# PolyU-IOR/HPR-LP-C

Measured on AMD Instinct MI355X. Metric: HPR iterations/sec (FP64), higher is better.
Workload: dtype f64

## Files before the change

hpr-lp-c_amd/csrc/abi.cpp:

```cpp
#include <algorithm>
#include <cmath>
#include <cstdlib>
#include <cstring>
#include <memory>
#include <mutex>
#include <iomanip>
#include <iostream>

#include "hprlp_amd.h"
#include "env.h"
#include "dist.h"
#include "presolve.h"
#include "reorder.h"
#include "solver.h"
#include "many.h"
#include "version.h"

using namespace hprlp;

struct hprlp_solver {
    Solver s;
    Comm *comm = nullptr;
    Comm *xcomm = nullptr;
    bool sharded = false;
// ... 1345 lines not shown
    return M.passes;
    GUARD_END(-1)
}

extern "C" int hprlp_tiled_host_check(int m, int n, const int *rowptr, const int *col, int R, int T, double min_dense, long out[6]) {
    try {
        if (m <= 0 || n <= 0 || !rowptr || !col || !out) throw std::runtime_error("bad arguments");
        tiled_host_check(m, n, rowptr, col, R, T, min_dense, out);
        return 0;
    } catch (const std::exception &e) {
        set_last_error(e.what());
        return -1;
    }
}

extern "C" int hprlp_env_switches(char *buf, int cap) {
    int count = 0;
    const EnvEntry *t = env_table(&count);
    std::string d;
    for (int i = 0; i < count; ++i) d += std::string(t[i].name) + "\t" + (t[i].kind == EnvKind::Integrator ? "integrator" : "hook") + "\t" + t[i].what + "\n";
    if (buf && cap > 0) std::snprintf(buf, static_cast<size_t>(cap), "%s", d.c_str());
    return static_cast<int>(d.size());
}

extern "C" int hprlp_solver_time_iterations(hprlp_solver *h, int warmup, int steps, int mode, double *total_ms,
                                            double *xhalf_ms, double *yhalf_ms) {
    GUARD_BEGIN
    Solver &s = h->s;
    if (steps <= 0) throw std::runtime_error("steps must be positive");
    s.run_normal(warmup);
// ... 61 lines not shown
```

hpr-lp-c_amd/csrc/env.cpp:

```cpp
#include "env.h"

#include <cstdlib>
#include <cstring>
#include <stdexcept>

namespace hprlp {

static const EnvEntry kTable[] = {
    {"HPRLP_TEST_HOOKS", EnvKind::Integrator, "1: honour the test hooks below (tests/conftest.py and the tools/ scripts set it)"},
    {"HPRLP_TIMING", EnvKind::Integrator, "wall time of the set-up and solve phases on stderr"},
    {"HPRLP_NO_GRAPH", EnvKind::Integrator, "launch normal iterations eagerly instead of replaying hipGraphs (fall-back)"},
    {"HPRLP_NO_TILED", EnvKind::Integrator, "never build the column-tiled matrix copies: stream kernel everywhere (fall-back)"},
    {"HPRLP_NO_REORDER", EnvKind::Integrator, "no set-up time locality ordering of a large matrix"},
    {"HPRLP_NO_ALLOC_CACHE", EnvKind::Integrator, "do not keep freed device blocks for the next solver of the process"},
    {"HPRLP_DIST_TRANSPORT", EnvKind::Integrator, "shm: hprlp_dist_unique_id names a shared-memory segment (host-staged group of processes on one node) instead of RCCL ids"},
    {"HPRLP_NO_WARM_MODEL", EnvKind::Integrator, "the model constructors do NOT start the HIP runtime / device context / code objects (for a process that forks workers after building its models: a HIP context does not survive fork); the first solve pays for them as in the reference"},
    {"HPRLP_DIST_EXCHANGE", EnvKind::Hook, "sparse | allgather: force the multi-GPU exchange form (same value on every rank)"},
    {"HPRLP_NO_OVERLAP", EnvKind::Integrator, "multi-GPU: shards unsplit, exchange in line on the solver stream"},
    {"HPRLP_DIST_TIMEOUT_S", EnvKind::Integrator, "seconds a rank of the shared-memory transport waits for its peers before it fails (default 120)"},
    {"HPRLP_BATCH_CHUNK", EnvKind::Hook, "solve_batched with 64 or more problems: chunk width of the panels (default 64; narrower chunks map one chunk to each XCD -- measured slower, profiles/r03_tiled_decomposition.md section 6b)"},
    {"HPRLP_BATCH_GRID", EnvKind::Hook, "solve_batched: cap on the row blocks of the normal half-step kernels (read at every call; a small cap makes every workgroup's row loop wrap)"},
    {"HPRLP_BATCH_LAMBDA", EnvKind::Hook, "solve_batched: the batch's lambda_max from the caller (strtod; hand it over as a C99 hex float to keep every bit) instead of 1.01 x the power iteration's estimate (read at every call)"},
    {"HPRLP_COPY_PAUSE_US", EnvKind::Hook, "piece size and pause of the threaded copies of set-up (64 MB, 100 us)"},
    {"HPRLP_COPY_PIECE_MB", EnvKind::Hook, "piece size and pause of the threaded copies of set-up (64 MB, 100 us)"},
// ... 28 lines not shown
    {"HPRLP_PRESOLVE_MAX_LINKS", EnvKind::Hook, "run one presolve stage alone / cut the chain after n links (tests, debugging)"},
    {"HPRLP_PRESOLVE_OFF", EnvKind::Hook, "switch presolve reductions / stages off (any subset; diagnostics)"},
    {"HPRLP_PRESOLVE_ONLY", EnvKind::Hook, "run one presolve stage alone / cut the chain after n links (tests, debugging)"},
    {"HPRLP_REORDER_CLUSTER", EnvKind::Hook, "knobs of the HOST reference path of the ordering (hprlp_locality_ordering): nodes per cluster, refinement sweeps, trimming percentage"},
    {"HPRLP_REORDER_HOST", EnvKind::Hook, "run the clustering of the locality ordering on the host (the reference form; default: on the device)"},
    {"HPRLP_REORDER_SWEEPS", EnvKind::Hook, "knobs of the HOST reference path of the ordering (hprlp_locality_ordering): nodes per cluster, refinement sweeps, trimming percentage"},
    {"HPRLP_REORDER_TRIM", EnvKind::Hook, "knobs of the HOST reference path of the ordering (hprlp_locality_ordering): nodes per cluster, refinement sweeps, trimming percentage"},
    {"HPRLP_SLACK_PIVOT", EnvKind::Hook, "pivot threshold of the costed slack-column substitution (default 0.5 of the row's largest entry)"},
    {"HPRLP_STORE_X", EnvKind::Hook, "every normal x-half reads and stores x (default for matrices with a tiled copy: inside a run of normal iterations x is rebuilt from x_hat and last_x by the next launch instead of travelling through memory)"},
    {"HPRLP_STREAM_NNZ", EnvKind::Hook, "row-block shape of the stream kernel (≤ 64 rows, ≤ 512 nonzeros per wave)"},
    {"HPRLP_STREAM_ROWS", EnvKind::Hook, "row-block shape of the stream kernel (≤ 64 rows, ≤ 512 nonzeros per wave)"},
    {"HPRLP_TILED_ANYWAY", EnvKind::Hook, "attempt the tiled form although neighbouring rows gather from the same lines (<= 0.25 lines per entry) / keep the piece form although an XCD's rows gather from under 3 MB"},
    {"HPRLP_TILED_MIN_COLS", EnvKind::Hook, "fewest columns for the tiled form (default 800 k, 2^19 for lowered super-blocks; 0 when HPRLP_TILED_MIN_ROWS is given)"},
    {"HPRLP_TILED_MIN_DENSE", EnvKind::Hook, "thresholds of the tiled copy (default 32·8192 rows, 0.5 of the entries in staged tiles)"},
    {"HPRLP_TILED_MIN_ROWS", EnvKind::Hook, "thresholds of the tiled copy (default 32·8192 rows, 0.5 of the entries in staged tiles)"},
    {"HPRLP_TILE_COLS", EnvKind::Hook, "force the tile width / super-block height of the tiled copies (default: Solver::choose_sb_rows)"},
    {"HPRLP_TILE_PIECES", EnvKind::Hook, "piece count of the tiled kernel's piece form (default: the chip's workgroup slots when the matrix has at most that many super-blocks; 0 = off)"},
    {"HPRLP_TILE_ROT", EnvKind::Hook, "alignment period of the rotated tile sweeps (default: mean window width of the matrix; 0 = ascending sweeps, i.e. CSR summation order)"},
    {"HPRLP_TILE_ROWS", EnvKind::Hook, "force the tile width / super-block height of the tiled copies (default: Solver::choose_sb_rows)"},
    {"HPRLP_TILE_STAMPS", EnvKind::Hook, "diagnostic instantiation of the piece kernel: shader-clock time per phase of a step on stderr when the solver is destroyed"},
    {"HPRLP_TILE_THREADS", EnvKind::Hook, "build the tiled copies with the host builder (background threads, default min(16, cores)) instead of on the device"},
    {"HPRLP_TILING_CHECK", EnvKind::Hook, "build them with both builders and fail on the first differing array element"},
    {"HPRLP_WG_TIMES", EnvKind::Hook, "diagnostic: per-workgroup wall-clock stamps of the fused tiled kernel on stderr"},
    {"HPRLP_WG_TIMES_DUMP", EnvKind::Hook, "per-workgroup stamps of the normal half-step kernels only, with the CU each ran on; raw table for tools/wgtimes_analyze.py"},
};

const EnvEntry *env_table(int *count) {
    if (count) *count = static_cast<int>(sizeof(kTable) / sizeof(kTable[0]));
    return kTable;
}
// ... 31 lines not shown
```

hpr-lp-c_amd/csrc/kernels.hip:

```cpp
#include "kernels.h"

#include <algorithm>
#include <vector>
#include <cmath>
#include <type_traits>

namespace hprlp {

__device__ __forceinline__ double wave_sum(double v) {
#pragma unroll
    for (int off = 32; off > 0; off >>= 1) v += __shfl_xor(v, off, kWave);
    return v;
}

__device__ __forceinline__ double wave_max(double v) {
#pragma unroll
    for (int off = 32; off > 0; off >>= 1) v = fmax(v, __shfl_xor(v, off, kWave));
    return v;
}

template <int NACC, int NW, int NMAX = 0>
__device__ __forceinline__ void block_store_partials_in(double (&acc)[NACC], double *partials, int stride, double (*red)[NACC > 0 ? NACC : 1]) {
    const int wave = threadIdx.x >> 6, lane = threadIdx.x & 63;
#pragma unroll
// ... 221 lines not shown
#ifndef HPRLP_EPI_NT
#define HPRLP_EPI_NT 2
#endif

template <int ED, int TD, bool REP, bool STAMP = false, bool LOGTERM = false, int TC = kTileCols>
__device__ __forceinline__ void tiled_sweep(const TiledDev &t, int s0, int nst, int first, int count, const double *__restrict__ vec,
                                            int ncols, double *acc, double *ytile, int tid, unsigned long long *stamp = nullptr) {
    constexpr int NT = kTileThreads, R = kTileRows, K = kTileChunk;
    constexpr int TPT = TC / NT;
    static_assert(TC == kTileCols || TC == kTileColsNarrow, "tile width");
    typedef double d2_t __attribute__((ext_vector_type(2)));
    const int lane = tid & 63;
    auto sidx = [&](int i) { i = min(i, count - 1) + first; return s0 + (i < nst ? i : i - nst); };
    int seg = 0, lim = 0;
    int tc0 = 0, tc1 = 0, tc2 = 0, tc3 = 0, tb0 = 0, tb1 = 0, tb2 = 0, tb3 = 0, te0 = 0, te1 = 0, te2 = 0, te3 = 0;
    auto getstep = [&](int k, int &col0, int &eb, int &ee) {
        const int r = min(k, lim - 1) - seg;
        col0 = step_field(tc0, tc1, tc2, tc3, r);
        eb = step_field(tb0, tb1, tb2, tb3, r);
        ee = step_field(te0, te1, te2, te3, r);
    };
    struct Ent {
        d2_t va, vb;
        uint32_t i0, i1, i2;
    };
    typedef uint32_t u3_t __attribute__((ext_vector_type(3), aligned(4)));
    auto issue_entries = [&](Ent &E, int k) {
        int col0, eb, ee_;
        getstep(k, col0, eb, ee_);
        const int e = eb + K * tid;
        const int ee = (e < ee_) ? e : eb;
        E.va = __builtin_nontemporal_load(reinterpret_cast<const d2_t *>(t.tval + ee));
        E.vb = __builtin_nontemporal_load(reinterpret_cast<const d2_t *>(t.tval + ee) + 1);
        const u3_t w = __builtin_nontemporal_load(reinterpret_cast<const u3_t *>(t.tidx3 + (ee / K) * 3));
        E.i0 = w.x;
        E.i1 = w.y;
        E.i2 = w.z;
    };
    typedef double d2u_t __attribute__((ext_vector_type(2), aligned(8)));
    auto issue_tile = [&](double (&tl)[TPT], int k) {
        int col0, eb, ee_;
        getstep(k, col0, eb, ee_);
        static_assert(TPT % 2 == 0, "tile loads come in pairs");
#pragma unroll
        for (int j = 0; j < TPT / 2; ++j) {
            const int p = col0 + 2 * (tid + j * NT);
            const int q = min(p, ncols - 2);
            d2u_t v = *reinterpret_cast<const d2u_t *>(vec + q);
            if (q != p) v.x = v.y;
            tl[2 * j] = v.x;
            tl[2 * j + 1] = v.y;
        }
    };
    auto store_tile = [&](const double (&tl)[TPT]) {
#pragma unroll
        for (int j = 0; j < TPT / 2; ++j) {
            d2_t v;
            v.x = tl[2 * j];
            v.y = tl[2 * j + 1];
            reinterpret_cast<d2_t *>(ytile)[tid + j * NT] = v;
        }
    };
    auto process = [&](const Ent &E, int k) {
        int col0, eb, ee_;
        getstep(k, col0, eb, ee_);
        if (K * tid < ee_ - eb) {
            const double v[K] = {E.va.x, E.va.y, E.vb.x, E.vb.y};
            const uint32_t c0 = E.i0, c1 = E.i1, c2 = E.i2;
            const uint32_t id[K] = {c0 & 0xffffffu, (c0 >> 24) | ((c1 & 0xffffu) << 8), (c1 >> 16) | ((c2 & 0xffu) << 16), c2 >> 8};
            uint32_t rw[K];
            double y[K];
#pragma unroll
            for (int k2 = 0; k2 < K; ++k2) {
                rw[k2] = id[k2] & (R - 1);
                y[k2] = ytile[id[k2] >> kTileRowBits];
            }
            double a[K];
#pragma unroll
            for (int k2 = 0; k2 < K; ++k2) a[k2] = acc[rw[k2]];
            double sk[K], pr[K];
#pragma unroll
            for (int k2 = 0; k2 < K; ++k2) pr[k2] = LOGTERM ? (v[k2] != v[k2] ? 0.0 : v[k2] - y[k2]) : v[k2] * y[k2];
            sk[0] = a[0] + pr[0];
#pragma unroll
// ... 2147 lines not shown
```

hpr-lp-c_amd/csrc/tiled.cpp:

```cpp
#include "tiled.h"
#include "env.h"

#include <algorithm>
#include <cstdlib>
#include <cstring>
#include <string>
#include <thread>
#include <type_traits>

namespace hprlp {

namespace {

struct Local {
    std::vector<int> sb_steps, sb_mid;
    std::vector<TileStep> steps;
    std::vector<char> step_is_rem;
    std::vector<uint32_t> tidx;
    std::vector<int> tperm, rcol, rperm;
    std::vector<uint16_t> rrow;
    long dense = 0, pad = 0;
};

void build_range(int rows, int cols, const int *rp, const int *ci, int sb0, int sb1, Local *L, int R, int T, int rem_cap) {
// ... 266 lines not shown
                if (row_of(k) != sb * R + rrow[e]) throw std::runtime_error("tiled check: a remainder entry in the wrong super-block / row");
            }
        }
    }
    for (long k = 0; k < nnz; ++k)
        if (!seen[k]) throw std::runtime_error("tiled check: an entry is missing");
    if (most_run > kTileLayers * ((static_cast<long>(R) * kTileChunk + kTileStepCap - 1) / kTileStepCap + 1)) throw std::runtime_error("tiled check: too many steps for one tile");
    out[0] = static_cast<long>(h.n_tile);
    out[1] = static_cast<long>(h.n_rem);
    out[2] = static_cast<long>(h.steps.size());
    out[3] = pads;
    out[4] = most_run;
    out[5] = static_cast<long>(1e6 * static_cast<double>(h.dense_entries) / static_cast<double>(nnz));
}

void DeviceTiled::upload(const TiledHost &h, int R, int T, int rem_cap) {
    n_tile = static_cast<long>(h.n_tile);
    n_rem = static_cast<long>(h.n_rem);
    n_steps = static_cast<int>(h.steps.size());
    const int nsb = static_cast<int>(h.sb_mid.size());
    sb_ptr.alloc(h.sb_ptr.size()); sb_ptr.upload(h.sb_ptr.data(), h.sb_ptr.size());
    sb_mid.alloc(h.sb_mid.size()); sb_mid.upload(h.sb_mid.data(), h.sb_mid.size());
    steps.alloc(h.steps.size()); steps.upload(h.steps.data(), h.steps.size());
    tidx.alloc_zero(h.n_tile + 8);
    tperm.alloc(h.n_tile + 8);
    tval.alloc_zero(h.n_tile + 8);
    rcol.alloc_zero(h.n_rem + 8);
    rperm.alloc(h.n_rem + 8);
    rrow.alloc_zero(h.n_rem + 8);
    size_t to = 0, ro = 0;
// ... 8 lines not shown
            HIP_CHECK(hipMemcpy(rrow.p + ro, pc.rrow.data(), pc.rrow.size() * sizeof(uint16_t), hipMemcpyHostToDevice));
        }
        to += pc.tidx.size();
        ro += pc.rcol.size();
    }
    view.valid = true;
    view.R = R;
    view.T = T;
    view.rem_cap = rem_cap;
    view.nsb = nsb;
    view.sb_ptr = sb_ptr.p;
    view.sb_mid = sb_mid.p;
    view.steps = steps.p;
    view.tval = tval.p;
    pack_indices(nullptr);
    view.tidx3 = tidx3.p;
    finish_schedule(nullptr);
}

void DeviceTiled::compare_with(const TiledHost &h) const {
    auto fail = [](const std::string &what) { throw std::runtime_error("tiling check: " + what); };
    if (n_tile != static_cast<long>(h.n_tile)) fail("tile entries " + std::to_string(n_tile) + " vs " + std::to_string(h.n_tile));
    if (n_rem != static_cast<long>(h.n_rem)) fail("remainder entries " + std::to_string(n_rem) + " vs " + std::to_string(h.n_rem));
    if (dense_entries != h.dense_entries || padding != h.padding) fail("dense / padding totals");
    auto same = [&](const char *name, const auto &dbuf, const auto &host) {
        using T = typename std::decay<decltype(host[0])>::type;
        std::vector<T> dev(host.size());
        if (!host.empty()) HIP_CHECK(hipMemcpy(dev.data(), dbuf.p, host.size() * sizeof(T), hipMemcpyDeviceToHost));
        for (size_t i = 0; i < host.size(); ++i)
            if (std::memcmp(&dev[i], &host[i], sizeof(T)) != 0) fail(std::string(name) + " differs at " + std::to_string(i));
    };
    same("sb_ptr", sb_ptr, h.sb_ptr);
    same("sb_mid", sb_mid, h.sb_mid);
    if (static_cast<size_t>(n_steps) != h.steps.size()) fail("step count");
    {
        std::vector<TileStep> dev(h.steps.size());
        if (!dev.empty()) HIP_CHECK(hipMemcpy(dev.data(), steps.p, dev.size() * sizeof(TileStep), hipMemcpyDeviceToHost));
        for (size_t i = 0; i < dev.size(); ++i)
            if (dev[i].col0 != h.steps[i].col0 || dev[i].e_begin != h.steps[i].e_begin || dev[i].e_end != h.steps[i].e_end)
                fail("steps differ at " + std::to_string(i));
    }
    std::vector<uint32_t> a_tidx;
    std::vector<int> a_tperm, a_rcol, a_rperm;
    std::vector<uint16_t> a_rrow;
    for (const TiledHost::Piece &pc : h.pieces) {
        a_tidx.insert(a_tidx.end(), pc.tidx.begin(), pc.tidx.end());
        a_tperm.insert(a_tperm.end(), pc.tperm.begin(), pc.tperm.end());
        a_rcol.insert(a_rcol.end(), pc.rcol.begin(), pc.rcol.end());
        a_rperm.insert(a_rperm.end(), pc.rperm.begin(), pc.rperm.end());
        a_rrow.insert(a_rrow.end(), pc.rrow.begin(), pc.rrow.end());
    }
    {
        std::vector<uint32_t> packed(a_tidx.size() / 4 * 3);
        for (size_t c = 0; c < a_tidx.size() / 4; ++c) {
            const uint32_t e0 = a_tidx[4 * c], e1 = a_tidx[4 * c + 1], e2 = a_tidx[4 * c + 2], e3 = a_tidx[4 * c + 3];
            packed[3 * c] = e0 | (e1 << 24);
            packed[3 * c + 1] = (e1 >> 8) | (e2 << 16);
            packed[3 * c + 2] = (e2 >> 16) | (e3 << 8);
        }
        same("tidx3", tidx3, packed);
    }
    same("tperm", tperm, a_tperm);
    same("rcol", rcol, a_rcol);
    same("rperm", rperm, a_rperm);
    same("rrow", rrow, a_rrow);
}

}
```

hpr-lp-c_amd/csrc/tiled.h:

```cpp
#pragma once

#include <hip/hip_runtime.h>

#include <cstdint>
#include <vector>

#include "common.h"

namespace hprlp {

constexpr int kTileThreads = 512;
constexpr int kTileRows = 8192;
constexpr int kTileCols = 2048;
constexpr int kTileColsNarrow = 1024;
constexpr int kTileChunk = 4;
constexpr int kTileStepCap = kTileThreads * kTileChunk;
constexpr int kTileRemK = 4;
constexpr int kTileRemCap = (kTileThreads - 4) * kTileRemK;
constexpr int kTileRemRun = 16;
#ifndef HPRLP_PB_REM_K
#define HPRLP_PB_REM_K 8
#endif
constexpr int kPbRemK = HPRLP_PB_REM_K;
constexpr int kPbRemCap = kTileThreads * kPbRemK;
constexpr int kPbRowsMax = 4096;
constexpr int kPbRunTabCap = 3072;
constexpr int kTileMaxRow = 1024;
constexpr int kTileDenseMin = 256;
static_assert(kTileRemCap % kTileRemK == 0 && kTileRemCap + (kTileThreads / 64) * 3 / 2 <= kTileCols, "tile buffer too small for the remainder scratch");
constexpr int kTileRowBits = 13;
constexpr int kTileRowsMin = 1024;
static_assert((1 << kTileRowBits) == kTileRows && kTileCols <= (1 << (24 - kTileRowBits)) && kTileChunk == 4,
              "entry codes are 24 bits: 13 of local row, 11 of local column, four per chunk");
inline uint32_t tile_code(int lcol, int row) { return (static_cast<uint32_t>(lcol) << kTileRowBits) | static_cast<uint32_t>(row); }

struct PackLayout {
    int n1 = 0, n2 = 0, n3 = 0, n4 = 0;
    int u3 = 0, u2 = 0, r1 = 0, c2 = 0;
    __host__ __device__ void set(int a1, int a2, int a3, int a4) {
        n1 = a1; n2 = a2; n3 = a3; n4 = a4;
        u3 = n1 < n3 ? n1 : n3;
        c2 = (n2 + 1) / 2;
        const int left = n1 - u3;
        u2 = (n2 & 1) ? (left < 2 ? left : 2) : 0;
        r1 = left - u2;
    }
    __host__ __device__ int entries() const { return kTileChunk * (n4 + n3 + c2 + (r1 + 3) / 4); }
    __host__ __device__ int pos(int L, int j) const {
        if (L == 4) return 4 * j;
// ... 58 lines not shown
    double *parts = nullptr;
    const int4 *side_blk = nullptr;
    int side_nblk = 0;
    const int4 *side_long = nullptr;
    int side_nlong = 0;
    double *side_partial = nullptr;
    const int *side_rows = nullptr;
    double *base = nullptr;
    unsigned long long *stamps = nullptr;
    unsigned long long *wgtimes = nullptr;
    int wg_filter = 0;
    const int *sb_ptr = nullptr;
    const int *sb_mid = nullptr;
    const TileStep *steps = nullptr;
    const double *tval = nullptr;
    const uint32_t *tidx3 = nullptr;
    double *P = nullptr;
    const uint32_t *rq = nullptr;
    int n_groups = 0;
    const int *f_gptr = nullptr;
    const double *f_val = nullptr;
    const int *f_pos = nullptr;
    const uint16_t *f_lcol = nullptr;
    const int *f_rptr = nullptr;
    const int *f_rk = nullptr;
    const int *f_rp = nullptr;
    int f_maxruns = 0;
    const int4 *f_work = nullptr;
    int n_work = 0;
};

// ... 5 lines not shown
        std::vector<int> tperm;
        std::vector<int> rcol, rperm;
        std::vector<uint16_t> rrow;
    };
    std::vector<Piece> pieces;
    size_t n_tile = 0, n_rem = 0;
    long dense_entries = 0;
    long padding = 0;
};

bool build_tiled(int rows, int cols, const int *rowptr, const int *col, TiledHost *out, int min_rows,
                 double min_dense_fraction, int R = kTileRows, int T = kTileCols, int rem_cap = kTileRemCap);

void tiled_host_check(int rows, int cols, const int *rp, const int *ci, int R, int T, double min_dense, long out[6]);

void compact_without_rows(long nnz, int rows, const int *rp_dev, const int *rp_c_dev, const int *col_dev, int *col_c, int *map_c, hipStream_t s);

struct DeviceTiled {
    DBuf<int> sb_ptr, sb_mid, tperm, rperm, rcol;
    DBuf<TileStep> steps;
    DBuf<uint32_t> tidx;
    DBuf<uint32_t> tidx3;
    DBuf<uint16_t> rrow;
    DBuf<double> tval;
    DBuf<double> P, f_val;
    DBuf<uint32_t> rq;
    DBuf<int> f_gptr, f_pos, f_perm;
    DBuf<int> f_rptr, f_rk, f_rp;
    DBuf<int4> f_work;
    DBuf<uint16_t> f_lcol;
    TiledDev view;
    long n_tile = 0, n_rem = 0;
    double rem_top_share = 0.0;
    long dense_entries = 0, padding = 0;
    int n_steps = 0;
    void upload(const TiledHost &h, int R = kTileRows, int T = kTileCols, int rem_cap = kTileRemCap);
    void pack_indices(hipStream_t s);
// ... 25 lines not shown
```

hpr-lp-c_amd/csrc/tiled_build.hip:

```cpp
#include <algorithm>
#include <functional>
#include <cstdlib>
#include <hipcub/hipcub.hpp>

#include <vector>

#include "common.h"
#include "env.h"
#include "kernels.h"
#include "tiled.h"

namespace hprlp {

namespace {

constexpr int K = kTileChunk;
constexpr int kRowBits = kTileRowBits;

__device__ __forceinline__ int row_of_entry(const int *__restrict__ rowptr, int rows, int k) {
    int lo = 0, hi = rows;
    while (hi - lo > 1) {
        const int mid = lo + ((hi - lo) >> 1);
        if (rowptr[mid] <= k) lo = mid;
        else hi = mid;
// ... 271 lines not shown
    rperm[e] = k;
    rcol[e] = col[k];
    rrow[e] = static_cast<uint16_t>(row_of_entry(rowptr, rows, k) % R);
}

__global__ void __launch_bounds__(kThreads) k_rem_steps(int nsb, int rem_cap, const int *__restrict__ sb_mid, const int *__restrict__ rem_before,
                                                       TileStep *__restrict__ steps) {
    const int sb = blockIdx.x * kThreads + threadIdx.x;
    if (sb >= nsb) return;
    const int b = rem_before[sb], e = rem_before[sb + 1];
    for (int p = b, j = 0; p < e; p += rem_cap, ++j) steps[sb_mid[sb] + j] = TileStep{0, p, min(e, p + rem_cap), 0};
}

inline unsigned grid_for(long n) { return static_cast<unsigned>((n + kThreads - 1) / kThreads); }

__global__ void __launch_bounds__(kThreads) k_pack_codes(long nchunk, const uint32_t *__restrict__ code, uint32_t *__restrict__ packed) {
    const long c = static_cast<long>(blockIdx.x) * kThreads + threadIdx.x;
    if (c >= nchunk) return;
    const uint32_t e0 = code[4 * c], e1 = code[4 * c + 1], e2 = code[4 * c + 2], e3 = code[4 * c + 3];
    packed[3 * c] = e0 | (e1 << 24);
    packed[3 * c + 1] = (e1 >> 8) | (e2 << 16);
    packed[3 * c + 2] = (e2 >> 16) | (e3 << 8);
}

}

void DeviceTiled::pack_indices(hipStream_t s) {
    const long nchunk = n_tile / K;
    tidx3.alloc_zero(static_cast<size_t>(nchunk) * 3 + 8);
    if (nchunk > 0) hipLaunchKernelGGL(k_pack_codes, dim3(grid_for(nchunk)), dim3(kThreads), 0, s, nchunk, tidx.p, tidx3.p);
    HIP_CHECK(hipStreamSynchronize(s));
    tidx.release();
}

namespace {

__global__ void __launch_bounds__(kThreads) k_window_widths(int nsb, int T, const int *__restrict__ sb_ptr, const int *__restrict__ sb_mid,
                                                           const TileStep *__restrict__ steps, unsigned long long *__restrict__ out) {
    const int sb = blockIdx.x * kThreads + threadIdx.x;
    if (sb >= nsb) return;
    const int s0 = sb_ptr[sb], smid = sb_mid[sb];
    if (s0 >= smid) return;
    const int w = (steps[smid - 1].col0 - steps[s0].col0) / T + 1;
    atomicAdd(out, static_cast<unsigned long long>(w));
    atomicAdd(out + 1, 1ull);
    int rep = 0;
    for (int s = s0 + 1; s < smid; ++s) rep += steps[s].col0 == steps[s - 1].col0;
    if (rep) atomicAdd(out + 2, static_cast<unsigned long long>(rep));
}

__global__ void __launch_bounds__(kThreads) k_rotation(int nsb, int period, int T, const int *__restrict__ sb_ptr, const int *__restrict__ sb_mid,
                                                      TileStep *__restrict__ steps) {
    const int sb = blockIdx.x * kThreads + threadIdx.x;
    if (sb >= nsb) return;
    const int s0 = sb_ptr[sb], smid = sb_mid[sb];
    if (s0 >= smid) return;
    const int nst = smid - s0;
    const int w0 = steps[s0].col0 / T;
    const long target = static_cast<long>((w0 + period - 1) / period) * period * T;
    int lo = 0, hi = nst;
    while (lo < hi) {
        const int mid = (lo + hi) >> 1;
// ... 236 lines not shown

    dense_entries = static_cast<long>(tot[0]);
    padding = static_cast<long>(tot[1]);
    n_steps = total_steps;
    view = TiledDev();
    view.valid = true;
    view.R = R;
    view.T = T;
    view.rem_cap = rem_cap;
    view.nsb = nsb;
    view.sb_ptr = sb_ptr.p;
    view.sb_mid = sb_mid.p;
    view.steps = steps.p;
    view.tval = tval.p;
    pack_indices(s);
    view.tidx3 = tidx3.p;
    finish_schedule(s);
    return true;
}


namespace {

__global__ void __launch_bounds__(kThreads) k_far_step_of(int nsb, const int *__restrict__ sb_ptr, const int *__restrict__ sb_mid,
                                                         TileStep *__restrict__ steps, const uint16_t *__restrict__ rrow,
                                                         int *__restrict__ step_of, int *__restrict__ sb_of, bool mark) {
    const int sb = blockIdx.x;
    if (sb >= nsb) return;
    for (int s = sb_mid[sb]; s < sb_ptr[sb + 1]; ++s) {
        const TileStep st = steps[s];
        if (threadIdx.x == 0) steps[s].col0 = 0;
// ... 414 lines not shown
```

hpr-lp-c_amd/hprlp.py:

```python
import ctypes as C
import os
import time
import weakref

import numpy as np

_HERE = os.path.dirname(os.path.abspath(__file__))
_ROOT = os.path.dirname(_HERE)
LIB_PATH = os.environ.get("HPRLP_LIB") or os.path.join(_ROOT, "lib", "libhprlp.so")

c_int_p = C.POINTER(C.c_int)
c_dbl_p = C.POINTER(C.c_double)


class CParameters(C.Structure):
    _fields_ = [
        ("max_iter", C.c_int), ("stop_tol", C.c_double), ("time_limit", C.c_double),
        ("device_number", C.c_int), ("check_iter", C.c_int),
        ("CUSPARSE_spmv", C.c_bool), ("autotune_verbose", C.c_bool), ("use_CR_scaling", C.c_bool),
        ("use_Ruiz_scaling", C.c_bool), ("use_Pock_Chambolle_scaling", C.c_bool),
        ("use_bc_scaling", C.c_bool), ("use_presolve", C.c_bool),
    ]


# ... 742 lines not shown
        out = (C.c_long * 8)()
        self._chk(lib().hprlp_solver_info(self.h, out))
        keys = ("m", "n", "nnz", "blocks_A", "blocks_AT", "grid_y", "grid_x", "tiled")
        d = dict(zip(keys, [int(v) for v in out]))
        d["reordered"] = bool(d["tiled"] & 8)
        d["tiled"] &= 7
        return d

    def describe(self):
        buf = C.create_string_buffer(2048)
        L = lib()
        L.hprlp_solver_describe.argtypes = [C.c_void_p, C.c_char_p, C.c_int]
        self._chk(L.hprlp_solver_describe(self.h, buf, 2048))
        return buf.value.decode()

    def form_facts(self):
        L = lib()
        L.hprlp_solver_form_facts.argtypes = [C.c_void_p, C.c_int, C.POINTER(CFormFacts)]
        out = {}
        for which, name in enumerate(("A", "A^T")):
            buf = (CFormFacts * 2)()
            n = L.hprlp_solver_form_facts(self.h, which, buf)
            self._chk(min(n, 0))
            out[name] = [_struct_dict(buf[i]) for i in range(n)]
        return out

    def run(self, max_trace=4096):
        res = CResults()
        trace = (CTraceRow * max_trace)()
        nt = C.c_int(0)
# ... 91 lines not shown
```

include/hprlp_amd.h:

```cpp
#ifndef HPRLP_AMD_H
#define HPRLP_AMD_H

#include "HPRLP.h"

#ifdef __cplusplus
extern "C" {
#endif

typedef struct hprlp_solver hprlp_solver;

typedef struct hprlp_trace_row {
    int iter, restart_flag;
    double err_Rp, err_Rd, primal_obj, dual_obj, gap, kkt, sigma, current_gap, lambda_max;
} hprlp_trace_row;

const char *hprlp_last_error(void);
const char *hprlp_backend(void);
int hprlp_warmup(int device);
int hprlp_warmup_seconds(double out[4]);

void hprlp_release_device_cache(void);
int hprlp_alloc_cache_selftest(void);

hprlp_solver *hprlp_solver_create(const LP_info_cpu *model, const HPRLP_parameters *param);
// ... 117 lines not shown
                                                   hprlp_local_group *group);

typedef struct hprlp_presolve hprlp_presolve;
hprlp_presolve *hprlp_presolve_run(const LP_info_cpu *model);
const LP_info_cpu *hprlp_presolve_reduced(const hprlp_presolve *p);
int hprlp_presolve_stats(const hprlp_presolve *p, int out[16]);
int hprlp_presolve_postsolve(const hprlp_presolve *p, const double *xr, const double *yr, const double *zr, double *x,
                             double *y, double *z);
int hprlp_presolve_forward(const hprlp_presolve *p, const double *x, const double *y, double *xr, double *yr);
void hprlp_presolve_free(hprlp_presolve *p);
int hprlp_original_kkt(const LP_info_cpu *model, const double *x, const double *y, const double *z, double out[5]);

int hprlp_locality_ordering(int m, int n, const int *rowptr, const int *col, int *row_new2old, int *col_new2old, double out[6]);
int hprlp_row_block_plan(int m, int n, const int *rowptr, const int *col, int with_cuts, long out[6]);
int hprlp_tiled_host_check(int m, int n, const int *rowptr, const int *col, int R, int T, double min_dense, long out[6]);

typedef struct hprlp_form_built {
    long ok;
    long n_pieces, dense_entries, n_rem;
    double rem_top_share;
} hprlp_form_built;
typedef struct hprlp_form_facts {
    long rows, cols, nnz, longest_row;
    double long_row_share;
    double line_density;
    double xcd_gather_bytes;
    long sb_rows, slots;
    double min_dense_override;
    long sharded;
    long heaviest_block;
// ... 14 lines not shown
} hprlp_form_hooks;
typedef struct hprlp_form_decision {
    int min_rows, min_cols;
    double min_dense;
    int route;
    int side_tried;
    int kept;
    int form;
    int why;
    int long_rows_alone;
    int all_remainder_wanted;
    char note[96];
} hprlp_form_decision;
int hprlp_form_select(const hprlp_form_facts *facts, const hprlp_form_hooks *hooks, hprlp_form_decision *out);
int hprlp_solver_form_facts(hprlp_solver *s, int which, hprlp_form_facts out[2]);

#ifdef __cplusplus
}
#endif
#endif
```

Measured before the change: 787.0.

## Compress tiled-matrix entry codes to 10 bytes per chunk where shapes fit

Replaces the 12-byte packed index triple per chunk of four entries with a split layout: an 8-byte lo/hi word plus a 2-byte word, and a 2-byte extra word read only for steps marked wide. A compact encoding stores four 11-bit local columns plus the row pattern (ascending small deltas, repeated rows, pairs) when it fits. Each step gets a wide flag in the low bit of col0. The goal is to cut index bytes streamed by the tiled SpMV, at the cost of extra decode ALU, more load instructions, and a per-step choice of mode.

```diff
diff --git a/hpr-lp-c_amd/csrc/abi.cpp b/hpr-lp-c_amd/csrc/abi.cpp
--- a/hpr-lp-c_amd/csrc/abi.cpp
+++ b/hpr-lp-c_amd/csrc/abi.cpp
@@ -1383,6 +1383,30 @@
     }
 }
 
+extern "C" int hprlp_tile_codes_host_check(int m, int n, const int *rowptr, const int *col, int R, int T, double min_dense, int force_wide, long out[5]) {
+    try {
+        if (m <= 0 || n <= 0 || !rowptr || !col || !out) throw std::runtime_error("bad arguments");
+        tile_codes_host_check(m, n, rowptr, col, R, T, min_dense, force_wide != 0, out);
+        return 0;
+    } catch (const std::exception &e) {
+        set_last_error(e.what());
+        return -1;
+    }
+}
+
+extern "C" int hprlp_solver_tile_codes(hprlp_solver *h, long out[8]) {
+    GUARD_BEGIN
+    if (!h || !out) throw std::runtime_error("null solver / output");
+    Solver &s = h->s;
+    s.finish_tiling();
+    for (int w = 0; w < 2; ++w) {
+        const DeviceMatrix &M = w ? s.AT : s.A;
+        for (int i = 0; i < 4; ++i) out[4 * w + i] = M.view.tiled.valid ? M.tiled.code_stats[i] : 0;
+    }
+    return 0;
+    GUARD_END(-1)
+}
+
 extern "C" int hprlp_env_switches(char *buf, int cap) {
     int count = 0;
     const EnvEntry *t = env_table(&count);
diff --git a/hpr-lp-c_amd/csrc/env.cpp b/hpr-lp-c_amd/csrc/env.cpp
--- a/hpr-lp-c_amd/csrc/env.cpp
+++ b/hpr-lp-c_amd/csrc/env.cpp
@@ -66,6 +66,7 @@
     {"HPRLP_TILED_MIN_COLS", EnvKind::Hook, "fewest columns for the tiled form (default 800 k, 2^19 for lowered super-blocks; 0 when HPRLP_TILED_MIN_ROWS is given)"},
     {"HPRLP_TILED_MIN_DENSE", EnvKind::Hook, "thresholds of the tiled copy (default 32·8192 rows, 0.5 of the entries in staged tiles)"},
     {"HPRLP_TILED_MIN_ROWS", EnvKind::Hook, "thresholds of the tiled copy (default 32·8192 rows, 0.5 of the entries in staged tiles)"},
+    {"HPRLP_TILE_CODES", EnvKind::Hook, "wide: every tile step of the tiled copies keeps the 12-byte codes per chunk of four (default: 10 bytes wherever all chunks of a step fit, tiled.h); read when a copy is built"},
     {"HPRLP_TILE_COLS", EnvKind::Hook, "force the tile width / super-block height of the tiled copies (default: Solver::choose_sb_rows)"},
     {"HPRLP_TILE_PIECES", EnvKind::Hook, "piece count of the tiled kernel's piece form (default: the chip's workgroup slots when the matrix has at most that many super-blocks; 0 = off)"},
     {"HPRLP_TILE_ROT", EnvKind::Hook, "alignment period of the rotated tile sweeps (default: mean window width of the matrix; 0 = ascending sweeps, i.e. CSR summation order)"},
diff --git a/hpr-lp-c_amd/csrc/kernels.hip b/hpr-lp-c_amd/csrc/kernels.hip
--- a/hpr-lp-c_amd/csrc/kernels.hip
+++ b/hpr-lp-c_amd/csrc/kernels.hip
@@ -259,28 +259,34 @@
     auto sidx = [&](int i) { i = min(i, count - 1) + first; return s0 + (i < nst ? i : i - nst); };
     int seg = 0, lim = 0;
     int tc0 = 0, tc1 = 0, tc2 = 0, tc3 = 0, tb0 = 0, tb1 = 0, tb2 = 0, tb3 = 0, te0 = 0, te1 = 0, te2 = 0, te3 = 0;
+    bool wide_ = false;
     auto getstep = [&](int k, int &col0, int &eb, int &ee) {
         const int r = min(k, lim - 1) - seg;
-        col0 = step_field(tc0, tc1, tc2, tc3, r);
+        const int c = step_field(tc0, tc1, tc2, tc3, r);
+        col0 = c & ~kTileStepWide;
+        wide_ = (c & kTileStepWide) != 0;
         eb = step_field(tb0, tb1, tb2, tb3, r);
         ee = step_field(te0, te1, te2, te3, r);
     };
     struct Ent {
         d2_t va, vb;
-        uint32_t i0, i1, i2;
-    };
-    typedef uint32_t u3_t __attribute__((ext_vector_type(3), aligned(4)));
+        uint32_t i0, i1, i2, i3;
+    };
+    typedef uint32_t u2_t __attribute__((ext_vector_type(2)));
     auto issue_entries = [&](Ent &E, int k) {
         int col0, eb, ee_;
         getstep(k, col0, eb, ee_);
+        const bool wide = wide_;
         const int e = eb + K * tid;
         const int ee = (e < ee_) ? e : eb;
+        const int ch = ee / K;
         E.va = __builtin_nontemporal_load(reinterpret_cast<const d2_t *>(t.tval + ee));
         E.vb = __builtin_nontemporal_load(reinterpret_cast<const d2_t *>(t.tval + ee) + 1);
-        const u3_t w = __builtin_nontemporal_load(reinterpret_cast<const u3_t *>(t.tidx3 + (ee / K) * 3));
+        const u2_t w = __builtin_nontemporal_load(reinterpret_cast<const u2_t *>(t.tcode8) + ch);
         E.i0 = w.x;
         E.i1 = w.y;
-        E.i2 = w.z;
+        E.i2 = __builtin_nontemporal_load(t.tcode2 + ch);
+        E.i3 = *(t.tcode2w + (wide ? ch : 0));
     };
     typedef double d2u_t __attribute__((ext_vector_type(2), aligned(8)));
     auto issue_tile = [&](double (&tl)[TPT], int k) {
@@ -309,10 +315,11 @@
     auto process = [&](const Ent &E, int k) {
         int col0, eb, ee_;
         getstep(k, col0, eb, ee_);
+        const bool wide = wide_;
         if (K * tid < ee_ - eb) {
             const double v[K] = {E.va.x, E.va.y, E.vb.x, E.vb.y};
-            const uint32_t c0 = E.i0, c1 = E.i1, c2 = E.i2;
-            const uint32_t id[K] = {c0 & 0xffffffu, (c0 >> 24) | ((c1 & 0xffffu) << 8), (c1 >> 16) | ((c2 & 0xffu) << 16), c2 >> 8};
+            uint32_t id[K];
+            tile_codes_decode(wide, E.i0, E.i1, E.i2, E.i3, id);
             uint32_t rw[K];
             double y[K];
 #pragma unroll
diff --git a/hpr-lp-c_amd/csrc/tiled.cpp b/hpr-lp-c_amd/csrc/tiled.cpp
--- a/hpr-lp-c_amd/csrc/tiled.cpp
+++ b/hpr-lp-c_amd/csrc/tiled.cpp
@@ -304,6 +304,71 @@
     out[5] = static_cast<long>(1e6 * static_cast<double>(h.dense_entries) / static_cast<double>(nnz));
 }
 
+void pack_codes_host(const std::vector<int> &sb_ptr, const std::vector<int> &sb_mid, const std::vector<TileStep> &steps, const std::vector<uint32_t> &tidx,
+                     bool force_wide, TileCodesHost *out) {
+    const size_t nchunk = tidx.size() / kTileChunk;
+    out->c8.assign(nchunk + 8, make_uint2(0, 0));
+    out->c2.assign(nchunk + 8, 0);
+    out->c2w.assign(nchunk + 8, 0);
+    out->wide.assign(steps.size(), 0);
+    for (long &v : out->stats) v = 0;
+    for (size_t sb = 0; sb < sb_mid.size(); ++sb) {
+        for (int s = sb_ptr[sb]; s < sb_mid[sb]; ++s) {
+            const TileStep &st = steps[s];
+            const int ch0 = st.e_begin / kTileChunk, ch1 = st.e_end / kTileChunk;
+            bool wide = force_wide;
+            uint32_t lo, hi, b, bw;
+            for (int c = ch0; c < ch1 && !wide; ++c) wide = !tile_codes_compact(&tidx[4 * static_cast<size_t>(c)], &lo, &hi, &b);
+            for (int c = ch0; c < ch1; ++c) {
+                bw = 0;
+                if (wide) tile_codes_wide(&tidx[4 * static_cast<size_t>(c)], &lo, &hi, &b, &bw);
+                else tile_codes_compact(&tidx[4 * static_cast<size_t>(c)], &lo, &hi, &b);
+                out->c8[c] = make_uint2(lo, hi);
+                out->c2[c] = static_cast<uint16_t>(b);
+                out->c2w[c] = static_cast<uint16_t>(bw);
+            }
+            out->wide[s] = wide ? 1 : 0;
+            out->stats[wide ? 1 : 0] += 1;
+            out->stats[wide ? 3 : 2] += st.e_end - st.e_begin;
+        }
+    }
+}
+
+void tile_codes_host_check(int rows, int cols, const int *rp, const int *ci, int R, int T, double min_dense, bool force_wide, long out[5]) {
+    TiledHost h;
+    if (!build_tiled(rows, cols, rp, ci, &h, 1, min_dense, R, T, kTileRemCap)) throw std::runtime_error("tile codes check: the build declined the pattern");
+    std::vector<uint32_t> tidx;
+    for (const TiledHost::Piece &pc : h.pieces) tidx.insert(tidx.end(), pc.tidx.begin(), pc.tidx.end());
+    TileCodesHost pk;
+    pack_codes_host(h.sb_ptr, h.sb_mid, h.steps, tidx, force_wide, &pk);
+    long unfit = 0;
+    for (size_t sb = 0; sb < h.sb_mid.size(); ++sb) {
+        for (int s = h.sb_ptr[sb]; s < h.sb_mid[sb]; ++s) {
+            const TileStep &st = h.steps[s];
+            if (st.col0 & kTileStepWide) throw std::runtime_error("tile codes check: a tile's first column is odd");
+            bool all_fit = true;
+            for (int c = st.e_begin / kTileChunk; c < st.e_end / kTileChunk; ++c) {
+                uint32_t id[4], lo, hi, b;
+                tile_codes_decode(pk.wide[s] != 0, pk.c8[c].x, pk.c8[c].y, pk.c2[c], pk.c2w[c], id);
+                for (int q = 0; q < 4; ++q)
+                    if (id[q] != tidx[4 * static_cast<size_t>(c) + q]) throw std::runtime_error("tile codes check: chunk " + std::to_string(c) + " decodes to other codes");
+                if (!tile_codes_compact(&tidx[4 * static_cast<size_t>(c)], &lo, &hi, &b)) {
+                    all_fit = false;
+                    ++unfit;
+                } else {
+                    tile_codes_decode(false, lo, hi, b, 0, id);
+                    for (int q = 0; q < 4; ++q)
+                        if (id[q] != tidx[4 * static_cast<size_t>(c) + q]) throw std::runtime_error("tile codes check: the compact form of chunk " + std::to_string(c) + " decodes to other codes");
+                }
+            }
+            if (!pk.wide[s] && !all_fit) throw std::runtime_error("tile codes check: a compact step holds a chunk without a compact form");
+            if (pk.wide[s] && all_fit && !force_wide) throw std::runtime_error("tile codes check: a step is wide although all its chunks fit");
+        }
+    }
+    for (int i = 0; i < 4; ++i) out[i] = pk.stats[i];
+    out[4] = unfit;
+}
+
 void DeviceTiled::upload(const TiledHost &h, int R, int T, int rem_cap) {
     n_tile = static_cast<long>(h.n_tile);
     n_rem = static_cast<long>(h.n_rem);
@@ -342,7 +407,6 @@
     view.steps = steps.p;
     view.tval = tval.p;
     pack_indices(nullptr);
-    view.tidx3 = tidx3.p;
     finish_schedule(nullptr);
 }
 
@@ -365,7 +429,7 @@
         std::vector<TileStep> dev(h.steps.size());
         if (!dev.empty()) HIP_CHECK(hipMemcpy(dev.data(), steps.p, dev.size() * sizeof(TileStep), hipMemcpyDeviceToHost));
         for (size_t i = 0; i < dev.size(); ++i)
-            if (dev[i].col0 != h.steps[i].col0 || dev[i].e_begin != h.steps[i].e_begin || dev[i].e_end != h.steps[i].e_end)
+            if ((dev[i].col0 & ~kTileStepWide) != h.steps[i].col0 || dev[i].e_begin != h.steps[i].e_begin || dev[i].e_end != h.steps[i].e_end)
                 fail("steps differ at " + std::to_string(i));
     }
     std::vector<uint32_t> a_tidx;
@@ -379,14 +443,22 @@
         a_rrow.insert(a_rrow.end(), pc.rrow.begin(), pc.rrow.end());
     }
     {
-        std::vector<uint32_t> packed(a_tidx.size() / 4 * 3);
-        for (size_t c = 0; c < a_tidx.size() / 4; ++c) {
-            const uint32_t e0 = a_tidx[4 * c], e1 = a_tidx[4 * c + 1], e2 = a_tidx[4 * c + 2], e3 = a_tidx[4 * c + 3];
-            packed[3 * c] = e0 | (e1 << 24);
-            packed[3 * c + 1] = (e1 >> 8) | (e2 << 16);
-            packed[3 * c + 2] = (e2 >> 16) | (e3 << 8);
-        }
-        same("tidx3", tidx3, packed);
+        TileCodesHost pk;
+        const char *e = env_get("HPRLP_TILE_CODES");
+        pack_codes_host(h.sb_ptr, h.sb_mid, h.steps, a_tidx, e && std::strcmp(e, "wide") == 0, &pk);
+        pk.c8.resize(a_tidx.size() / 4);
+        pk.c2.resize(a_tidx.size() / 4);
+        pk.c2w.resize(a_tidx.size() / 4);
+        same("tcode8", tcode8, pk.c8);
+        same("tcode2", tcode2, pk.c2);
+        same("tcode2w", tcode2w, pk.c2w);
+        std::vector<TileStep> dev(h.steps.size());
+        if (!dev.empty()) HIP_CHECK(hipMemcpy(dev.data(), steps.p, dev.size() * sizeof(TileStep), hipMemcpyDeviceToHost));
+        for (size_t sb = 0; sb < h.sb_mid.size(); ++sb)
+            for (int q = h.sb_ptr[sb]; q < h.sb_mid[sb]; ++q)
+                if ((dev[q].col0 & kTileStepWide) != (pk.wide[q] ? kTileStepWide : 0)) fail("code mode of step " + std::to_string(q));
+        for (int i = 0; i < 4; ++i)
+            if (code_stats[i] != pk.stats[i]) fail("code statistics");
     }
     same("tperm", tperm, a_tperm);
     same("rcol", rcol, a_rcol);
diff --git a/hpr-lp-c_amd/csrc/tiled.h b/hpr-lp-c_amd/csrc/tiled.h
--- a/hpr-lp-c_amd/csrc/tiled.h
+++ b/hpr-lp-c_amd/csrc/tiled.h
@@ -33,6 +33,61 @@
 static_assert((1 << kTileRowBits) == kTileRows && kTileCols <= (1 << (24 - kTileRowBits)) && kTileChunk == 4,
               "entry codes are 24 bits: 13 of local row, 11 of local column, four per chunk");
 inline uint32_t tile_code(int lcol, int row) { return (static_cast<uint32_t>(lcol) << kTileRowBits) | static_cast<uint32_t>(row); }
+
+constexpr int kTileStepWide = 1;
+__host__ __device__ inline bool tile_codes_compact(const uint32_t e[4], uint32_t *lo, uint32_t *hi, uint32_t *b) {
+    constexpr uint32_t RM = (1u << kTileRowBits) - 1;
+    const uint32_t r0 = e[0] & RM, r1 = e[1] & RM, r2 = e[2] & RM, r3 = e[3] & RM;
+    const uint32_t c0 = e[0] >> kTileRowBits, c1 = e[1] >> kTileRowBits, c2 = e[2] >> kTileRowBits, c3 = e[3] >> kTileRowBits;
+    uint32_t shape, X;
+    if (r1 >= r0 && r1 - r0 < 128 && r2 >= r1 && r2 - r1 < 128 && r3 >= r2 && r3 - r2 < 128) {
+        shape = 0;
+        X = (r1 - r0) | (r2 - r1) << 7 | (r3 - r2) << 14;
+    } else if (r2 == r3 && (r1 == r0 || r1 == r2)) {
+        shape = 1;
+        X = r3 | (r1 != r0 ? 1u : (r2 != r1 ? 2u : 3u)) << 13;
+    } else if (r1 == r0 && r3 >= r2 && r3 - r2 < 256) {
+        shape = 2;
+        X = r2 | (r3 - r2) << 13;
+    } else if (r1 == r0 && r2 == r0) {
+        shape = 1;
+        X = r3 | 3u << 13;
+    } else {
+        return false;
+    }
+    *lo = c0 | c1 << 11 | (c2 & 1023u) << 22;
+    *hi = c2 >> 10 | c3 << 1 | shape << 12 | r0 << 14 | (X & 31u) << 27;
+    *b = X >> 5;
+    return true;
+}
+__host__ __device__ inline void tile_codes_wide(const uint32_t e[4], uint32_t *lo, uint32_t *hi, uint32_t *b, uint32_t *bw) {
+    const uint32_t w2 = (e[2] >> 16) | (e[3] << 8);
+    *lo = e[0] | (e[1] << 24);
+    *hi = (e[1] >> 8) | (e[2] << 16);
+    *b = w2 & 0xffffu;
+    *bw = w2 >> 16;
+}
+__host__ __device__ inline void tile_codes_decode(bool wide, uint32_t lo, uint32_t hi, uint32_t b, uint32_t bw, uint32_t id[4]) {
+    if (wide) {
+        const uint32_t w2 = b | (bw << 16);
+        id[0] = lo & 0xffffffu;
+        id[1] = (lo >> 24) | ((hi & 0xffffu) << 8);
+        id[2] = (hi >> 16) | ((w2 & 0xffu) << 16);
+        id[3] = w2 >> 8;
+        return;
+    }
+    constexpr uint32_t RM = (1u << kTileRowBits) - 1;
+    const uint32_t shape = (hi >> 12) & 3u, r0 = (hi >> 14) & RM, X = (hi >> 27) | (b << 5);
+    const uint32_t ra = X & RM, y = X >> kTileRowBits;
+    const uint32_t k = shape == 1 ? y : 2u, d = shape == 1 ? 0u : y;
+    const uint32_t q1 = r0 + (X & 127u), q2 = q1 + ((X >> 7) & 127u), q3 = q2 + (X >> 14);
+    const bool run = shape == 0;
+    const uint32_t w1 = run ? q1 : (k > 1 ? r0 : ra), w2 = run ? q2 : (k > 2 ? r0 : ra), w3 = run ? q3 : ra + d;
+    id[0] = ((lo & 2047u) << kTileRowBits) | r0;
+    id[1] = (((lo >> 11) & 2047u) << kTileRowBits) | w1;
+    id[2] = (((lo >> 22) | ((hi & 1u) << 10)) << kTileRowBits) | w2;
+    id[3] = (((hi >> 1) & 2047u) << kTileRowBits) | w3;
+}
 
 struct PackLayout {
     int n1 = 0, n2 = 0, n3 = 0, n4 = 0;
@@ -121,7 +176,9 @@
     const int *sb_mid = nullptr;
     const TileStep *steps = nullptr;
     const double *tval = nullptr;
-    const uint32_t *tidx3 = nullptr;
+    const uint2 *tcode8 = nullptr;
+    const uint16_t *tcode2 = nullptr;
+    const uint16_t *tcode2w = nullptr;
     double *P = nullptr;
     const uint32_t *rq = nullptr;
     int n_groups = 0;
@@ -157,13 +214,25 @@
 
 void tiled_host_check(int rows, int cols, const int *rp, const int *ci, int R, int T, double min_dense, long out[6]);
 
+struct TileCodesHost {
+    std::vector<uint2> c8;
+    std::vector<uint16_t> c2, c2w;
+    std::vector<char> wide;
+    long stats[4] = {0, 0, 0, 0};
+};
+void pack_codes_host(const std::vector<int> &sb_ptr, const std::vector<int> &sb_mid, const std::vector<TileStep> &steps, const std::vector<uint32_t> &tidx,
+                     bool force_wide, TileCodesHost *out);
+void tile_codes_host_check(int rows, int cols, const int *rp, const int *ci, int R, int T, double min_dense, bool force_wide, long out[5]);
+
 void compact_without_rows(long nnz, int rows, const int *rp_dev, const int *rp_c_dev, const int *col_dev, int *col_c, int *map_c, hipStream_t s);
 
 struct DeviceTiled {
     DBuf<int> sb_ptr, sb_mid, tperm, rperm, rcol;
     DBuf<TileStep> steps;
     DBuf<uint32_t> tidx;
-    DBuf<uint32_t> tidx3;
+    DBuf<uint2> tcode8;
+    DBuf<uint16_t> tcode2, tcode2w;
+    long code_stats[4] = {0, 0, 0, 0};
     DBuf<uint16_t> rrow;
     DBuf<double> tval;
     DBuf<double> P, f_val;
diff --git a/hpr-lp-c_amd/csrc/tiled_build.hip b/hpr-lp-c_amd/csrc/tiled_build.hip
--- a/hpr-lp-c_amd/csrc/tiled_build.hip
+++ b/hpr-lp-c_amd/csrc/tiled_build.hip
@@ -1,6 +1,7 @@
 #include <algorithm>
 #include <functional>
 #include <cstdlib>
+#include <cstring>
 #include <hipcub/hipcub.hpp>
 
 #include <vector>
@@ -309,23 +310,63 @@
 
 inline unsigned grid_for(long n) { return static_cast<unsigned>((n + kThreads - 1) / kThreads); }
 
-__global__ void __launch_bounds__(kThreads) k_pack_codes(long nchunk, const uint32_t *__restrict__ code, uint32_t *__restrict__ packed) {
-    const long c = static_cast<long>(blockIdx.x) * kThreads + threadIdx.x;
-    if (c >= nchunk) return;
-    const uint32_t e0 = code[4 * c], e1 = code[4 * c + 1], e2 = code[4 * c + 2], e3 = code[4 * c + 3];
-    packed[3 * c] = e0 | (e1 << 24);
-    packed[3 * c + 1] = (e1 >> 8) | (e2 << 16);
-    packed[3 * c + 2] = (e2 >> 16) | (e3 << 8);
+__global__ void __launch_bounds__(kThreads) k_pack_codes(int nsb, const int *__restrict__ sb_ptr, const int *__restrict__ sb_mid, TileStep *__restrict__ steps,
+                                                        const uint32_t *__restrict__ code, uint2 *__restrict__ c8, uint16_t *__restrict__ c2,
+                                                        uint16_t *__restrict__ c2w, int force_wide, unsigned long long *__restrict__ stats) {
+    const int sb = blockIdx.x;
+    if (sb >= nsb) return;
+    unsigned long long n_steps[2] = {0, 0}, n_ent[2] = {0, 0};
+    for (int s = sb_ptr[sb]; s < sb_mid[sb]; ++s) {
+        const TileStep st = steps[s];
+        const int ch0 = st.e_begin / K, ch1 = st.e_end / K;
+        int bad = force_wide;
+        for (int c = ch0 + threadIdx.x; c < ch1 && !bad; c += kThreads) {
+            uint32_t lo, hi, b;
+            bad = !tile_codes_compact(code + 4 * static_cast<long>(c), &lo, &hi, &b);
+        }
+        const int wide = __syncthreads_or(bad) ? 1 : 0;
+        for (int c = ch0 + threadIdx.x; c < ch1; c += kThreads) {
+            uint32_t lo, hi, b, bw = 0;
+            if (wide) tile_codes_wide(code + 4 * static_cast<long>(c), &lo, &hi, &b, &bw);
+            else tile_codes_compact(code + 4 * static_cast<long>(c), &lo, &hi, &b);
+            c8[c] = make_uint2(lo, hi);
+            c2[c] = static_cast<uint16_t>(b);
+            c2w[c] = static_cast<uint16_t>(bw);
+        }
+        if (threadIdx.x == 0) steps[s].col0 = (st.col0 & ~kTileStepWide) | (wide ? kTileStepWide : 0);
+        n_steps[wide] += 1;
+        n_ent[wide] += static_cast<unsigned long long>(st.e_end - st.e_begin);
+    }
+    if (threadIdx.x == 0) {
+        atomicAdd(stats, n_steps[0]);
+        atomicAdd(stats + 1, n_steps[1]);
+        atomicAdd(stats + 2, n_ent[0]);
+        atomicAdd(stats + 3, n_ent[1]);
+    }
 }
 
 }
 
 void DeviceTiled::pack_indices(hipStream_t s) {
     const long nchunk = n_tile / K;
-    tidx3.alloc_zero(static_cast<size_t>(nchunk) * 3 + 8);
-    if (nchunk > 0) hipLaunchKernelGGL(k_pack_codes, dim3(grid_for(nchunk)), dim3(kThreads), 0, s, nchunk, tidx.p, tidx3.p);
+    tcode8.alloc_zero(static_cast<size_t>(nchunk) + 8);
+    tcode2.alloc_zero(static_cast<size_t>(nchunk) + 8);
+    tcode2w.alloc_zero(static_cast<size_t>(nchunk) + 8);
+    const char *e = env_get("HPRLP_TILE_CODES");
+    const int force_wide = (e && std::strcmp(e, "wide") == 0) ? 1 : 0;
+    DBuf<unsigned long long> stats;
+    stats.alloc_zero(4);
+    if (view.nsb > 0 && nchunk > 0)
+        hipLaunchKernelGGL(k_pack_codes, dim3(view.nsb), dim3(kThreads), 0, s, view.nsb, sb_ptr.p, sb_mid.p, steps.p, tidx.p, tcode8.p, tcode2.p, tcode2w.p,
+                           force_wide, stats.p);
     HIP_CHECK(hipStreamSynchronize(s));
+    unsigned long long h[4] = {0, 0, 0, 0};
+    stats.download(h, 4);
+    for (int i = 0; i < 4; ++i) code_stats[i] = static_cast<long>(h[i]);
     tidx.release();
+    view.tcode8 = tcode8.p;
+    view.tcode2 = tcode2.p;
+    view.tcode2w = tcode2w.p;
 }
 
 namespace {
@@ -340,7 +381,7 @@
     atomicAdd(out, static_cast<unsigned long long>(w));
     atomicAdd(out + 1, 1ull);
     int rep = 0;
-    for (int s = s0 + 1; s < smid; ++s) rep += steps[s].col0 == steps[s - 1].col0;
+    for (int s = s0 + 1; s < smid; ++s) rep += (steps[s].col0 & ~kTileStepWide) == (steps[s - 1].col0 & ~kTileStepWide);
     if (rep) atomicAdd(out + 2, static_cast<unsigned long long>(rep));
 }
 
@@ -607,7 +648,6 @@
     view.steps = steps.p;
     view.tval = tval.p;
     pack_indices(s);
-    view.tidx3 = tidx3.p;
     finish_schedule(s);
     return true;
 }
diff --git a/hpr-lp-c_amd/hprlp.py b/hpr-lp-c_amd/hprlp.py
--- a/hpr-lp-c_amd/hprlp.py
+++ b/hpr-lp-c_amd/hprlp.py
@@ -780,6 +780,18 @@
         self._chk(L.hprlp_solver_describe(self.h, buf, 2048))
         return buf.value.decode()
 
+    def tile_codes(self):
+        L = lib()
+        L.hprlp_solver_tile_codes.argtypes = [C.c_void_p, C.POINTER(C.c_long)]
+        out = (C.c_long * 8)()
+        self._chk(L.hprlp_solver_tile_codes(self.h, out))
+        res = {}
+        for w, name in enumerate(("A", "A^T")):
+            cs, ws, ce, we = (int(v) for v in out[4 * w:4 * w + 4])
+            res[name] = {"compact_steps": cs, "wide_steps": ws, "compact_entries": ce, "wide_entries": we,
+                         "compact_share": ce / (ce + we) if ce + we else 0.0}
+        return res
+
     def form_facts(self):
         L = lib()
         L.hprlp_solver_form_facts.argtypes = [C.c_void_p, C.c_int, C.POINTER(CFormFacts)]
diff --git a/include/hprlp_amd.h b/include/hprlp_amd.h
--- a/include/hprlp_amd.h
+++ b/include/hprlp_amd.h
@@ -155,6 +155,7 @@
 int hprlp_locality_ordering(int m, int n, const int *rowptr, const int *col, int *row_new2old, int *col_new2old, double out[6]);
 int hprlp_row_block_plan(int m, int n, const int *rowptr, const int *col, int with_cuts, long out[6]);
 int hprlp_tiled_host_check(int m, int n, const int *rowptr, const int *col, int R, int T, double min_dense, long out[6]);
+int hprlp_tile_codes_host_check(int m, int n, const int *rowptr, const int *col, int R, int T, double min_dense, int force_wide, long out[5]);
 
 typedef struct hprlp_form_built {
     long ok;
@@ -199,6 +200,7 @@
 } hprlp_form_decision;
 int hprlp_form_select(const hprlp_form_facts *facts, const hprlp_form_hooks *hooks, hprlp_form_decision *out);
 int hprlp_solver_form_facts(hprlp_solver *s, int which, hprlp_form_facts out[2]);
+int hprlp_solver_tile_codes(hprlp_solver *s, long out[8]);
 
 #ifdef __cplusplus
 }
```

Measured after the change: 775.6. -1.4%, worse.
